# PufferAI/PufferLib

Measured on AMD Instinct MI355X. Metric: env steps/sec end-to-end PPO (rollout+GAE+update), 4096 envs, higher is better.
Workload: dtype f32; 1 GPU; squared d=3 nt=1, 4096 envs/GPU x 128 steps, obs 49->64 f32 rows, MLP 128, 4 minibatches x 4 epochs, bptt 16 (BASELINE configs[1]); global_batch=524288, parallelism=dp1

## Files before the change

### pufferlib_amd/csrc/lane_ops.hpp

```cpp
#pragma once
#include "common.hpp"

namespace pfa {

template <int CTRL>
__device__ __forceinline__ float dpp_f(float x) {
    return __int_as_float(__builtin_amdgcn_update_dpp(0, __float_as_int(x), CTRL, 0xf, 0xf, false));
}
template <int CTRL>
__device__ __forceinline__ int dpp_i(int x) {
    return __builtin_amdgcn_update_dpp(0, x, CTRL, 0xf, 0xf, false);
}

constexpr int kDppXor1 = 0xB1;
constexpr int kDppXor2 = 0x4E;
constexpr int kDppHalfMirror = 0x141;
constexpr int kDppMirror = 0x140;

__device__ __forceinline__ float row16_max(float x) {
    x = fmaxf(x, dpp_f<kDppXor1>(x));
    x = fmaxf(x, dpp_f<kDppXor2>(x));
    x = fmaxf(x, dpp_f<kDppHalfMirror>(x));
    x = fmaxf(x, dpp_f<kDppMirror>(x));
    return x;
}

__device__ __forceinline__ float row16_sum(float x) {
    x = x + dpp_f<kDppXor1>(x);
    x = x + dpp_f<kDppXor2>(x);
    x = x + dpp_f<kDppHalfMirror>(x);
    x = x + dpp_f<kDppMirror>(x);
    return x;
}

__device__ __forceinline__ void row16_argmax(float &best, int &idx) {
#define PFA_ARGMAX_STEP(CTRL)                                   \
    {                                                           \
        const float ob = dpp_f<CTRL>(best);                     \
        const int oi = dpp_i<CTRL>(idx);                        \
        const bool take = (ob > best) | ((ob == best) & (oi < idx));  \
        best = take ? ob : best;                                \
        idx = take ? oi : idx;                                  \
    }
    PFA_ARGMAX_STEP(kDppXor1)
    PFA_ARGMAX_STEP(kDppXor2)
    PFA_ARGMAX_STEP(kDppHalfMirror)
    PFA_ARGMAX_STEP(kDppMirror)
#undef PFA_ARGMAX_STEP
}

}
```

### pufferlib_amd/csrc/rollout.hip

```cpp
#include "common.hpp"
#include "lane_ops.hpp"
#include "mlp_tile.hpp"
#include "philox.hpp"
#include "rollout_tile.hpp"
#include "sampler.hpp"
#include "squared_env.hpp"

namespace pfa {

#ifdef PFA_PROBES
__device__ unsigned long long *g_rtrace = nullptr;
__device__ int g_rtrace_t0 = 0, g_rtrace_steps = 0;
#define PFA_RSTAMP(t, k)                                                                                            \
    do {                                                                                                            \
        if (g_rtrace && blockIdx.x == 0 && (threadIdx.x & 63) == 0 && (t) >= g_rtrace_t0 && (t) < g_rtrace_t0 + g_rtrace_steps) \
            g_rtrace[(((size_t)(threadIdx.x >> 6)) * g_rtrace_steps + ((t) - g_rtrace_t0)) * 8 + (k)] = __builtin_amdgcn_s_memtime(); \
    } while (0)
#else
#define PFA_RSTAMP(t, k) do { } while (0)
#endif

template <int DP, int KS, int MW = kMW>
__global__ void __launch_bounds__(kRollThreads) mlp_forward_sample_kernel(const float *obs, long long rows, MlpView pv,
                                                                         int a, uint32_t heads, const float *noise,
                                                                         uint64_t seed, uint64_t step, long long row_offset,
                                                                         long long *actions, float *logprob, float *entropy,
                                                                         float *value) {
    __shared__ float xs[XTile<DP>::kFloats];
    __shared__ float part[kRollWaves][kPartFloats];
    SliceFrags<DP, KS, MW> w;
    w.load(pv);
    const int le = threadIdx.x >> 4, lo = threadIdx.x & 15;
    const long long tiles = (rows + 15) / 16;
    for (long long tile = blockIdx.x; tile < tiles; tile += gridDim.x) {
        __syncthreads();
        stage_rows<DP>(obs, tile * 16, rows, xs);
        __syncthreads();
        forward_slice<DP, KS, MW>(w, xs, part);
        __syncthreads();
        const long long row = tile * 16 + le;
        const bool ok = row < rows;
        const float q = ok ? noise_lane(noise ? noise + row * a : nullptr, seed, step, (uint64_t)(row_offset + row), lo, a) : 1.0f;
        const LaneSample sm = heads ? sample_lanes_heads(part, le, lo, a, heads, q) : sample_lanes(part, le, lo, a, q);
        if (ok && lo == 0) {
            actions[row] = sm.action;
            logprob[row] = sm.logprob;
            if (entropy) entropy[row] = sm.entropy;
            value[row] = sm.value;
        }
    }
}

template <int DP, int EPW, bool NT1, int KS, int MW = kMW>
__global__ void __launch_bounds__(kRollThreads) rollout_mlp_squared_kernel(SquaredView v, MlpView pv, int a,
                                                                          pfa_experience ex, const float *noise,
                                                                          uint64_t seed, uint64_t step0, long long env_offset,
                                                                          float *live_obs, float *live_rew, uint8_t *live_term,
                                                                          uint8_t *live_trunc, uint8_t *live_mask) {
    constexpr int XS = XTile<DP>::XS;
    __shared__ float xs[XTile<DP>::kFloats];
    __shared__ float part[kRollWaves][kPartFloats];
    __shared__ uint16_t tg[NT1 ? 1 : 16 * kMaxTargets];
    __builtin_amdgcn_s_setprio(3);
    __shared__ RewardTable rtab;
    const int le = threadIdx.x >> 4, lo = threadIdx.x & 15;
    const int e = blockIdx.x * EPW + le;
    const bool env_ok = le < EPW && e < v.n;
    const bool owner = lo == 0 && env_ok;
    const int T = ex.horizon_T;

    SliceFrags<DP, KS, MW> w;
    w.load(pv);

    stage_rows<DP>(live_obs, (long long)blockIdx.x * EPW, v.n, xs, EPW);
    if (NT1) rtab.build(v.d);
    SquaredEnv s;
    Target1 t1;
    float reward = 0.0f;
    bool terminal = false;
    long long filled = 0;
    uint16_t next_cell = 0;
    uint32_t slot = 0;
    const size_t tape_n = (size_t)v.n;
    if (owner) {
        squared_load(v, e, s);
        if (NT1) {
            t1.set(v.tgt[e], v.g);
            filled = v.hdr->rounds_filled;
            slot = s.rounds % (uint32_t)v.tape_rounds;
            next_cell = v.tape[(size_t)slot * tape_n + e];
        } else {
            for (int t = 0; t < v.nt; ++t) tg[le * kMaxTargets + t] = v.tgt[(size_t)t * v.n + e];
        }
        reward = live_rew[e];
        terminal = live_term[e] != 0;
    }
    const bool noise_lane_ok = env_ok && lo < a;
    const float *nz = noise && noise_lane_ok ? noise + (size_t)e * a + lo : nullptr;
    const size_t nz_step = (size_t)v.n * a;
    float q_next = nz ? nz[0] : 1.0f;
    __builtin_amdgcn_s_waitcnt(0x0F70);
    __syncthreads();

    for (int t = 0; t < T; ++t) {
        PFA_RSTAMP(t, 0);
        unstage_rows<DP>(xs, ex.obs + (size_t)t * DP, (long long)blockIdx.x * EPW, v.n, (size_t)T * DP, EPW);
        PFA_RSTAMP(t, 1);
        forward_slice<DP, KS, MW>(w, xs, part);
        PFA_RSTAMP(t, 2);
        lds_barrier();
        PFA_RSTAMP(t, 3);
        const float q = noise ? q_next
                              : (env_ok ? noise_lane(nullptr, seed, step0 + t, (uint64_t)(env_offset + e), lo, a) : 1.0f);
#ifdef PFA_PROBES
        if (q == -12345.678f) PFA_RSTAMP(t, 7);
#endif
        PFA_RSTAMP(t, 4);
        const LaneSample sm = sample_lanes(part, le, lo, a, q);
#ifdef PFA_PROBES
        if (sm.value == 12345.678f) PFA_RSTAMP(t, 7);
#endif
        PFA_RSTAMP(t, 5);
        if (owner) {
            const float stored_reward = reward;
            const bool stored_terminal = terminal;
            float *grid = xs + le * XS;
            if (NT1) {
                if (s.done) {
                    if ((long long)s.rounds >= filled) v.hdr->underrun = 1;
                    squared_reset_nt1(v, s, grid, t1, next_cell, reward, terminal);
                    s.rounds += 1;
                    slot = slot + 1 == (uint32_t)v.tape_rounds ? 0u : slot + 1;
                } else {
                    squared_step_nt1(v, s, grid, t1, rtab, sm.action, reward, terminal);
                }
            } else {
                uint16_t *tc = tg + le * kMaxTargets;
                if (s.done) {
                    if ((long long)s.rounds >= v.hdr->rounds_filled) v.hdr->underrun = 1;
                    const uint16_t *tr = v.tape + (size_t)(s.rounds % (uint32_t)v.tape_rounds) * v.nt * v.n;
                    squared_reset(v, e, s, grid, tr, tc, reward, terminal);
                    s.rounds += 1;
                } else {
                    bool fin;
                    double fr, fs;
                    int fl;
                    squared_step(v, s, grid, tc, sm.action, reward, terminal, fin, fr, fl, fs);
                }
            }
            const size_t row = (size_t)e * T + t;
            ex.rewards[row] = stored_reward;
            ex.dones[row] = stored_terminal ? 1.0f : 0.0f;
            ex.actions[row] = sm.action;
            ex.logprobs[row] = sm.logprob;
            ex.values[row] = sm.value;
            if (NT1) next_cell = v.tape[(size_t)slot * tape_n + e];
        }
        if (nz && t + 1 < T) q_next = nz[(size_t)(t + 1) * nz_step];
        PFA_RSTAMP(t, 6);
        lds_barrier();
        PFA_RSTAMP(t, 7);
    }

    if (owner) {
        squared_store(v, e, s);
        if (NT1) {
            v.tgt[e] = t1.cell;
        } else {
            for (int t = 0; t < v.nt; ++t) v.tgt[(size_t)t * v.n + e] = tg[le * kMaxTargets + t];
        }
        v.fin[e] = 0;
        live_rew[e] = reward;
        live_term[e] = terminal ? 1 : 0;
        live_trunc[e] = 0;
        live_mask[e] = 1;
    }
    unstage_rows<DP>(xs, live_obs, (long long)blockIdx.x * EPW, v.n, (size_t)DP, EPW);
}

__global__ void __launch_bounds__(256) philox_exp_noise_kernel(float *out, long long steps, long long rows, int a, int groups,
                                                               uint64_t seed, uint64_t step0, long long row_offset) {
    const long long total = steps * rows * groups;
    for (long long i = (long long)blockIdx.x * blockDim.x + threadIdx.x; i < total; i += (long long)gridDim.x * blockDim.x) {
        const int j4 = (int)(i % groups);
        const long long tr = i / groups;
        const long long r = tr % rows, t = tr / rows;
        const uint64_t step = step0 + (uint64_t)t, row = (uint64_t)(row_offset + r);
        const u32x4 w = philox4x32_10((uint32_t)row, (uint32_t)j4, (uint32_t)step, (uint32_t)(step >> 32), (uint32_t)seed,
                                      (uint32_t)(seed >> 32));
        float *o = out + (size_t)tr * a + 4 * j4;
        const int left = a - 4 * j4;
        o[0] = -logf(philox_uniform(w.x));
        if (left > 1) o[1] = -logf(philox_uniform(w.y));
        if (left > 2) o[2] = -logf(philox_uniform(w.z));
        if (left > 3) o[3] = -logf(philox_uniform(w.w));
    }
}

struct TilePolicy {
    MlpView pv;
    int obs_dim, obs_stride;
    uint32_t heads;
};

static int check_shape(bool flat, int hidden, int obs_dim, int obs_stride, int a, uint32_t heads) {
    if (flat) {
        PFA_REQUIRE(hidden == kHidden, "mlp: hidden must be %d (got %d)", kHidden, hidden);
    } else {
        PFA_REQUIRE(hidden == 64 || hidden == 128 || hidden == 256 || hidden == 512, "mlp view: hidden %d is not one of 64/128/256/512", hidden);
    }
    PFA_REQUIRE(obs_stride == 16 || obs_stride == 32 || obs_stride == 64 || (flat && (obs_stride == 96 || obs_stride == 128)),
                "mlp: obs_stride must be one of %s (got %d)", flat ? "16/32/64/96/128" : "16/32/64", obs_stride);
    PFA_REQUIRE(obs_dim >= 1 && obs_dim <= obs_stride, "mlp: obs_dim %d out of range", obs_dim);
    PFA_REQUIRE(a >= 1 && a <= 15, "mlp: num_actions must be in 1..15 (got %d)", a);
    PFA_REQUIRE(heads == 0 || (flat && heads_count(heads, a) >= 1), "mlp: head sizes 0x%x do not sum to num_actions %d", heads, a);
    return 0;
}
static int check_dims(const pfa_mlp_dims *d) {
    PFA_REQUIRE(d != nullptr, "mlp: null dims");
    return check_shape(true, d->hidden, d->obs_dim, d->obs_stride, d->num_actions, d->heads);
}
static int check_view(const pfa_mlp_view *p) {
    PFA_REQUIRE(p != nullptr, "mlp view: null");
    PFA_REQUIRE(p->w1 && p->b1 && p->w2 && p->b2 && p->wv && p->bv, "mlp view: null tensor");
    PFA_REQUIRE(p->ldw1 >= p->obs_dim, "mlp view: obs_dim %d / ldw1 %d out of range", p->obs_dim, p->ldw1);
    return check_shape(false, p->hidden, p->obs_dim, p->obs_stride, p->num_actions, 0);
}
static int policy_of_flat(const float *params, const pfa_mlp_dims *d, TilePolicy *out) {
    if (int rc = check_dims(d)) return rc;
    PFA_REQUIRE(params, "mlp: null parameter buffer");
    *out = TilePolicy{mlp_view_of_flat(params, d->obs_stride, d->num_actions), d->obs_dim, d->obs_stride, d->heads};
    return 0;
}
static int policy_of_view(const pfa_mlp_view *p, TilePolicy *out) {
    if (int rc = check_view(p)) return rc;
    *out = TilePolicy{MlpView{p->w1, p->ldw1, p->obs_dim, p->b1, p->w2, p->b2, p->wv, p->bv, p->num_actions, p->hidden}, p->obs_dim,
                      p->obs_stride, 0};
    return 0;
}

template <int DP_, int KS_, int MW_>
struct Tile {
    static constexpr int DP = DP_, KS = KS_, MW = MW_;
};
template <int MW, class Launch>
static void dispatch_stride(const TilePolicy &p, Launch launch) {
    if (p.obs_stride == 64 && p.obs_dim > 48 && p.obs_dim <= 52) return launch(Tile<64, 13, MW>{});
    switch (p.obs_stride) {
        case 16: return launch(Tile<16, 4, MW>{});
        case 32: return launch(Tile<32, 8, MW>{});
        case 64: return launch(Tile<64, 16, MW>{});
    }
    if constexpr (MW == kMW) {
        if (p.obs_stride == 96) return launch(Tile<96, 24, MW>{});
        return launch(Tile<128, 32, MW>{});
    }
}
template <class Launch>
static void dispatch_tile(const TilePolicy &p, Launch launch) {
    switch (p.pv.hidden) {
        case 64: return dispatch_stride<1>(p, launch);
        case 128: return dispatch_stride<2>(p, launch);
        case 256: return dispatch_stride<4>(p, launch);
        default: return dispatch_stride<8>(p, launch);
    }
}

static int launch_forward_sample(const TilePolicy &p, const float *obs, int64_t rows, const float *noise, const pfa_noise_key *key,
                                 int64_t row_offset, int64_t *actions, float *logprob, float *entropy, float *value, pfa_stream_t stream) {
    PFA_REQUIRE(rows >= 0, "mlp.forward: negative rows");
    if (rows == 0) return 0;
    PFA_REQUIRE(obs && actions && logprob && value, "mlp.forward: null buffer");
    PFA_REQUIRE(noise || key, "mlp.forward: need an explicit noise tensor or a Philox key");
    const uint64_t seed = key ? key->seed : 0, step = key ? key->step : 0;
    const int64_t tiles = (rows + 15) / 16;
    const unsigned grid = (unsigned)(tiles < 4096 ? tiles : 4096);
    dispatch_tile(p, [&](auto tile) {
        using T = decltype(tile);
        hipLaunchKernelGGL((mlp_forward_sample_kernel<T::DP, T::KS, T::MW>), dim3(grid), dim3(kRollThreads), 0, (hipStream_t)stream, obs,
                           (long long)rows, p.pv, p.pv.a, p.heads, noise, seed, step, (long long)row_offset, (long long *)actions, logprob,
                           entropy, value);
    });
    PFA_LAUNCH_CHECK();
    return 0;
}

static int launch_rollout_squared(const TilePolicy &p, void *state, const pfa_squared_config *cfg, const pfa_experience *exp,
                                  const float *noise, const pfa_noise_key *key, int64_t env_offset, float *obs, float *rewards,
                                  uint8_t *terminals, uint8_t *truncations, uint8_t *masks, pfa_stream_t stream) {
    PFA_REQUIRE(state && cfg && exp && obs && rewards && terminals && truncations && masks, "rollout: null buffer");
    PFA_REQUIRE(p.heads == 0, "rollout: the fused rollout samples one Discrete head");
    PFA_REQUIRE(cfg->obs_stride == p.obs_stride, "rollout: env obs_stride %d != policy obs_stride %d", cfg->obs_stride, p.obs_stride);
    PFA_REQUIRE(exp->horizon_T >= 1, "rollout: horizon must be >= 1");
    PFA_REQUIRE(exp->obs && exp->actions && exp->logprobs && exp->values && exp->rewards && exp->dones,
                "rollout: null experience buffer");
    PFA_REQUIRE(noise || key, "rollout: need an explicit noise tensor or a Philox key");
    PFA_REQUIRE(cfg->num_targets <= kMaxTargets, "rollout: too many targets");
    SquaredView v = squared_view(state, *cfg);
    const uint64_t seed = key ? key->seed : 0, step = key ? key->step : 0;
    ScopedKernelTimer timer("rollout_mlp_squared", (hipStream_t)stream);
    const unsigned grid = (unsigned)((cfg->num_envs + 15) / 16);
    const bool nt1 = cfg->num_targets == 1;
    dispatch_tile(p, [&](auto tile) {
        using T = decltype(tile);
        auto *kernel = nt1 ? rollout_mlp_squared_kernel<T::DP, 16, true, T::KS, T::MW> : rollout_mlp_squared_kernel<T::DP, 16, false, T::KS, T::MW>;
        hipLaunchKernelGGL(kernel, dim3(grid), dim3(kRollThreads), 0, (hipStream_t)stream, v, p.pv, p.pv.a, *exp, noise, seed, step,
                           (long long)env_offset, obs, rewards, terminals, truncations, masks);
    });
    PFA_LAUNCH_CHECK();
    return 0;
}

}

using namespace pfa;

#ifdef PFA_PROBES
extern "C" int pfa_probe_set_rollout_trace(unsigned long long *buf, int t0, int steps) {
    PFA_CHECK_HIP(hipMemcpyToSymbol(HIP_SYMBOL(g_rtrace), &buf, sizeof(buf)));
    PFA_CHECK_HIP(hipMemcpyToSymbol(HIP_SYMBOL(g_rtrace_t0), &t0, sizeof(t0)));
    PFA_CHECK_HIP(hipMemcpyToSymbol(HIP_SYMBOL(g_rtrace_steps), &steps, sizeof(steps)));
    return 0;
}
#endif

extern "C" int64_t pfa_mlp_param_count(const pfa_mlp_dims *dims) {
    if (check_dims(dims)) return -1;
    return mlp_offsets(dims->obs_stride, dims->num_actions).count;
}

extern "C" int pfa_mlp_forward_sample(const float *obs, int64_t rows, const float *params, const pfa_mlp_dims *dims,
                                      const float *noise, const pfa_noise_key *key, int64_t row_offset, int64_t *actions,
                                      float *logprob, float *entropy, float *value, pfa_stream_t stream) {
    TilePolicy p;
    if (int rc = policy_of_flat(params, dims, &p)) return rc;
    return launch_forward_sample(p, obs, rows, noise, key, row_offset, actions, logprob, entropy, value, stream);
}

extern "C" int pfa_mlp_view_supported(const pfa_mlp_view *p) { return check_view(p) == 0 ? 1 : 0; }

extern "C" int pfa_mlp_view_forward_sample(const float *obs, int64_t rows, const pfa_mlp_view *view, const float *noise,
                                           const pfa_noise_key *key, int64_t row_offset, int64_t *actions, float *logprob,
                                           float *entropy, float *value, pfa_stream_t stream) {
    TilePolicy p;
    if (int rc = policy_of_view(view, &p)) return rc;
    return launch_forward_sample(p, obs, rows, noise, key, row_offset, actions, logprob, entropy, value, stream);
}

extern "C" int pfa_philox_exp_noise(float *out, int64_t steps, int64_t rows, int32_t num_actions, const pfa_noise_key *key,
                                    int64_t row_offset, pfa_stream_t stream) {
    PFA_REQUIRE(steps >= 0 && rows >= 0, "philox noise: negative shape");
    PFA_REQUIRE(num_actions >= 1 && num_actions <= 15, "philox noise: num_actions must be in 1..15 (got %d)", num_actions);
    if (steps == 0 || rows == 0) return 0;
    PFA_REQUIRE(out && key, "philox noise: null buffer");
    const int groups = (num_actions + 3) / 4;
    const long long total = (long long)steps * rows * groups;
    const unsigned grid = (unsigned)((total + 255) / 256 < 65536 ? (total + 255) / 256 : 65536);
    ScopedKernelTimer timer("philox_exp_noise", (hipStream_t)stream);
    hipLaunchKernelGGL(philox_exp_noise_kernel, dim3(grid), dim3(256), 0, (hipStream_t)stream, out, (long long)steps, (long long)rows,
                       (int)num_actions, groups, key->seed, key->step, (long long)row_offset);
    PFA_LAUNCH_CHECK();
    return 0;
}

extern "C" int pfa_rollout_mlp_squared(void *state, const pfa_squared_config *cfg, const float *params,
                                       const pfa_mlp_dims *dims, const pfa_experience *exp, const float *noise,
                                       const pfa_noise_key *key, int64_t env_offset, float *obs, float *rewards,
                                       uint8_t *terminals, uint8_t *truncations, uint8_t *masks, pfa_stream_t stream) {
    TilePolicy p;
    if (int rc = policy_of_flat(params, dims, &p)) return rc;
    return launch_rollout_squared(p, state, cfg, exp, noise, key, env_offset, obs, rewards, terminals, truncations, masks, stream);
}

extern "C" int pfa_rollout_mlp_view_squared(void *state, const pfa_squared_config *cfg, const pfa_mlp_view *view, const pfa_experience *exp,
                                            const float *noise, const pfa_noise_key *key, int64_t env_offset, float *obs, float *rewards,
                                            uint8_t *terminals, uint8_t *truncations, uint8_t *masks, pfa_stream_t stream) {
    TilePolicy p;
    if (int rc = policy_of_view(view, &p)) return rc;
    return launch_rollout_squared(p, state, cfg, exp, noise, key, env_offset, obs, rewards, terminals, truncations, masks, stream);
}
```

### pufferlib_amd/csrc/rollout_tile.hpp

```cpp
#pragma once
#include "common.hpp"
#include "lane_ops.hpp"
#include "mlp_tile.hpp"
#include "philox.hpp"
#include "sampler.hpp"

namespace pfa {

constexpr int kRollThreads = 256;
constexpr int kRollWaves = 4;
constexpr int kMW = kMT / kRollWaves;

struct MlpView {
    const float *w1;
    int ldw1, cols;
    const float *b1;
    const float *w2;
    const float *b2;
    const float *wv;
    const float *bv;
    int a, hidden;
    __device__ __forceinline__ float w2v(int o, int u) const { return o < a ? w2[o * hidden + u] : (o == a ? wv[u] : 0.0f); }
    __device__ __forceinline__ float b2v(int o) const { return o < a ? b2[o] : (o == a ? bv[0] : 0.0f); }
};
inline MlpView mlp_view_of_flat(const float *params, int dp, int a) {
    const MlpOffsets off = mlp_offsets(dp, a);
    return MlpView{params + off.w1, dp, dp, params + off.b1, params + off.w2, params + off.b2, params + off.wv, params + off.bv, a, kHidden};
}

template <int DP, int KS = DP / 4, int MW = kMW>
struct SliceFrags {
    float w1f[MW][KS], b1f[MW][4], w2f[MW][4], bo[4];
    __device__ __forceinline__ void load(const float *params, int a) {
        const MlpOffsets off = mlp_offsets(DP, a);
        const int wv = wave_id(), c = lane_id() & 15, g = lane_id() >> 4;
#pragma unroll
        for (int i = 0; i < MW; ++i) {
            const int m = MW * wv + i;
#pragma unroll
            for (int kk = 0; kk < KS; ++kk) w1f[i][kk] = params[off.w1 + (16 * m + c) * DP + 4 * kk + g];
#pragma unroll
            for (int r = 0; r < 4; ++r) {
                b1f[i][r] = params[off.b1 + 16 * m + 4 * g + r];
                w2f[i][r] = w2v_at(params, off, a, c, 16 * m + 4 * g + r);
            }
        }
#pragma unroll
        for (int r = 0; r < 4; ++r) bo[r] = wv == 0 ? b2v_at(params, off, a, 4 * g + r) : 0.0f;
    }
    __device__ __forceinline__ void load(const MlpView &p) {
        const int wv = wave_id(), c = lane_id() & 15, g = lane_id() >> 4;
#pragma unroll
        for (int i = 0; i < MW; ++i) {
            const int m = MW * wv + i;
#pragma unroll
            for (int kk = 0; kk < KS; ++kk) w1f[i][kk] = 4 * kk + g < p.cols ? p.w1[(size_t)(16 * m + c) * p.ldw1 + 4 * kk + g] : 0.0f;
#pragma unroll
            for (int r = 0; r < 4; ++r) {
                b1f[i][r] = p.b1[16 * m + 4 * g + r];
                w2f[i][r] = p.w2v(c, 16 * m + 4 * g + r);
            }
        }
#pragma unroll
        for (int r = 0; r < 4; ++r) bo[r] = wv == 0 ? p.b2v(4 * g + r) : 0.0f;
    }
};

template <int DP>
__device__ __forceinline__ void stage_rows(const float *src, long long first_row, long long rows, float *xs,
                                           int tile_rows = 16) {
    constexpr int XS = XTile<DP>::XS, V = DP / 4;
    for (int idx = threadIdx.x; idx < 16 * V; idx += kRollThreads) {
        const int r = idx / V, c4 = idx - r * V;
        float4 x = make_float4(0.f, 0.f, 0.f, 0.f);
        if (r < tile_rows && first_row + r < rows) x = *reinterpret_cast<const float4 *>(src + (first_row + r) * DP + 4 * c4);
        float2 *d = reinterpret_cast<float2 *>(xs + r * XS + 4 * c4);
        d[0] = make_float2(x.x, x.y);
        d[1] = make_float2(x.z, x.w);
    }
}

template <int DP>
__device__ __forceinline__ void unstage_rows(const float *xs, float *dst, long long first_row, long long rows, size_t row_stride,
                                             int tile_rows = 16) {
    constexpr int XS = XTile<DP>::XS, V = DP / 4;
    for (int idx = threadIdx.x; idx < tile_rows * V; idx += kRollThreads) {
        const int r = idx / V, c4 = idx - r * V;
        if (first_row + r < rows) {
            const float2 *sp = reinterpret_cast<const float2 *>(xs + r * XS + 4 * c4);
            const float2 lo2 = sp[0], hi2 = sp[1];
            *reinterpret_cast<float4 *>(dst + (size_t)(first_row + r) * row_stride + 4 * c4) = make_float4(lo2.x, lo2.y, hi2.x, hi2.y);
        }
    }
}

template <int DP, int KS = DP / 4, int MW = kMW>
__device__ __forceinline__ void forward_slice(const SliceFrags<DP, KS, MW> &w, const float *xs, float (*part)[kPartFloats]) {
    constexpr int XS = XTile<DP>::XS;
    const int wv = wave_id(), c = lane_id() & 15, g = lane_id() >> 4;
    f32x4 h[MW];
#pragma unroll
    for (int i = 0; i < MW; ++i) h[i] = f32x4{w.b1f[i][0], w.b1f[i][1], w.b1f[i][2], w.b1f[i][3]};
    float bv[KS];
#pragma unroll
    for (int kk = 0; kk < KS; ++kk) bv[kk] = xs[c * XS + 4 * kk + g];
    __builtin_amdgcn_sched_barrier(0);
#pragma unroll
    for (int kk = 0; kk < KS; ++kk) {
#pragma unroll
        for (int i = 0; i < MW; ++i) h[i] = mfma16(w.w1f[i][kk], bv[kk], h[i]);
    }
    f32x4 o0 = f32x4{w.bo[0], w.bo[1], w.bo[2], w.bo[3]}, o1 = f32x4{0.f, 0.f, 0.f, 0.f};
#pragma unroll
    for (int i = 0; i < MW; i += 2) {
#pragma unroll
        for (int r = 0; r < 4; ++r) {
            o0 = mfma16(w.w2f[i][r], fmaxf(h[i][r], 0.0f), o0);
            if constexpr (MW >= 2) o1 = mfma16(w.w2f[i + 1][r], fmaxf(h[i + 1][r], 0.0f), o1);
        }
    }
    const f32x4 po = o0 + o1;
#pragma unroll
    for (int r = 0; r < 4; ++r) part[wv][(4 * g + r) * kPartStride + c] = po[r];
}

__device__ __forceinline__ LaneSample sample_lanes(const float (*part)[kPartFloats], int le, int lo, int a, float q) {
    const int i = lo * kPartStride + le;
    const float mine = (part[0][i] + part[1][i]) + (part[2][i] + part[3][i]);
    return sample_row16(mine, lo, a, q);
}
__device__ __forceinline__ LaneSample sample_lanes_heads(const float (*part)[kPartFloats], int le, int lo, int a, uint32_t heads, float q) {
    const int i = lo * kPartStride + le;
    const float mine = (part[0][i] + part[1][i]) + (part[2][i] + part[3][i]);
    return sample_row16_heads(mine, lo, a, heads, q);
}

}
```

Measured before the change: 422.1 million env_steps/s.

## Overlap obs unstaging with first-layer MFMAs and tighten DPP/relu lane ops

The per-step obs write-out (LDS to global) is split into a load phase issued alongside the activation reads and a store phase placed inside the first-layer MFMA loop between sched barriers. The goal is to hide global-store issue behind matrix work rather than run it serially before the forward pass. It also replaces update_dpp with mov_dpp using bound_ctrl, rewrites row16_max as inline fused v_max_f32_dpp asm with s_nops, and computes ReLU as an integer max on the float bits. The inline asm and the integer ReLU change handling of NaN and negative zero, and the extra staged registers can raise register pressure.

After: 426.3 million env_steps/s, median of 6. Within noise of the previous version (+1.0%).

```diff
diff --git a/pufferlib_amd/csrc/lane_ops.hpp b/pufferlib_amd/csrc/lane_ops.hpp
--- a/pufferlib_amd/csrc/lane_ops.hpp
+++ b/pufferlib_amd/csrc/lane_ops.hpp
@@ -5,11 +5,11 @@
 
 template <int CTRL>
 __device__ __forceinline__ float dpp_f(float x) {
-    return __int_as_float(__builtin_amdgcn_update_dpp(0, __float_as_int(x), CTRL, 0xf, 0xf, false));
+    return __int_as_float(__builtin_amdgcn_mov_dpp(__float_as_int(x), CTRL, 0xf, 0xf, true));
 }
 template <int CTRL>
 __device__ __forceinline__ int dpp_i(int x) {
-    return __builtin_amdgcn_update_dpp(0, x, CTRL, 0xf, 0xf, false);
+    return __builtin_amdgcn_mov_dpp(x, CTRL, 0xf, 0xf, true);
 }
 
 constexpr int kDppXor1 = 0xB1;
@@ -18,10 +18,16 @@
 constexpr int kDppMirror = 0x140;
 
 __device__ __forceinline__ float row16_max(float x) {
-    x = fmaxf(x, dpp_f<kDppXor1>(x));
-    x = fmaxf(x, dpp_f<kDppXor2>(x));
-    x = fmaxf(x, dpp_f<kDppHalfMirror>(x));
-    x = fmaxf(x, dpp_f<kDppMirror>(x));
+    asm("s_nop 1\n\t"
+        "v_max_f32_dpp %0, %0, %0 quad_perm:[1,0,3,2] row_mask:0xf bank_mask:0xf bound_ctrl:1\n\t"
+        "s_nop 1\n\t"
+        "v_max_f32_dpp %0, %0, %0 quad_perm:[2,3,0,1] row_mask:0xf bank_mask:0xf bound_ctrl:1\n\t"
+        "s_nop 1\n\t"
+        "v_max_f32_dpp %0, %0, %0 row_half_mirror row_mask:0xf bank_mask:0xf bound_ctrl:1\n\t"
+        "s_nop 1\n\t"
+        "v_max_f32_dpp %0, %0, %0 row_mirror row_mask:0xf bank_mask:0xf bound_ctrl:1\n\t"
+        "s_nop 1"
+        : "+v"(x));
     return x;
 }
 
diff --git a/pufferlib_amd/csrc/rollout.hip b/pufferlib_amd/csrc/rollout.hip
--- a/pufferlib_amd/csrc/rollout.hip
+++ b/pufferlib_amd/csrc/rollout.hip
@@ -104,9 +104,9 @@
 
     for (int t = 0; t < T; ++t) {
         PFA_RSTAMP(t, 0);
-        unstage_rows<DP>(xs, ex.obs + (size_t)t * DP, (long long)blockIdx.x * EPW, v.n, (size_t)T * DP, EPW);
+        RowUnstage<DP> rows_out(xs, ex.obs + (size_t)t * DP, (long long)blockIdx.x * EPW, v.n, (size_t)T * DP, EPW);
         PFA_RSTAMP(t, 1);
-        forward_slice<DP, KS, MW>(w, xs, part);
+        forward_slice<DP, KS, MW>(w, xs, part, rows_out);
         PFA_RSTAMP(t, 2);
         lds_barrier();
         PFA_RSTAMP(t, 3);
diff --git a/pufferlib_amd/csrc/rollout_tile.hpp b/pufferlib_amd/csrc/rollout_tile.hpp
--- a/pufferlib_amd/csrc/rollout_tile.hpp
+++ b/pufferlib_amd/csrc/rollout_tile.hpp
@@ -1,4 +1,5 @@
 #pragma once
+#include <type_traits>
 #include "common.hpp"
 #include "lane_ops.hpp"
 #include "mlp_tile.hpp"
@@ -81,22 +82,53 @@
 }
 
 template <int DP>
+struct RowUnstage {
+    static constexpr int XS = XTile<DP>::XS, V = DP / 4, kPieces = (16 * V + kRollThreads - 1) / kRollThreads;
+    float *dst;
+    long long first_row, rows;
+    size_t row_stride;
+    int tile_rows;
+    const float *xs;
+    float2 lo2[kPieces], hi2[kPieces];
+    __device__ __forceinline__ RowUnstage(const float *xs_, float *dst_, long long first_row_, long long rows_, size_t row_stride_,
+                                          int tile_rows_ = 16)
+        : dst(dst_), first_row(first_row_), rows(rows_), row_stride(row_stride_), tile_rows(tile_rows_), xs(xs_) {}
+    __device__ __forceinline__ bool live(int idx, int r) const { return idx < tile_rows * V && first_row + r < rows; }
+    __device__ __forceinline__ void load() {
+#pragma unroll
+        for (int i = 0; i < kPieces; ++i) {
+            const int idx = threadIdx.x + i * kRollThreads, r = idx / V, c4 = idx - r * V;
+            if (live(idx, r)) {
+                const float2 *sp = reinterpret_cast<const float2 *>(xs + r * XS + 4 * c4);
+                lo2[i] = sp[0];
+                hi2[i] = sp[1];
+            }
+        }
+    }
+    __device__ __forceinline__ void store() const {
+#pragma unroll
+        for (int i = 0; i < kPieces; ++i) {
+            const int idx = threadIdx.x + i * kRollThreads, r = idx / V, c4 = idx - r * V;
+            if (live(idx, r))
+                *reinterpret_cast<float4 *>(dst + (size_t)(first_row + r) * row_stride + 4 * c4) = make_float4(lo2[i].x, lo2[i].y, hi2[i].x, hi2[i].y);
+        }
+    }
+};
+template <int DP>
 __device__ __forceinline__ void unstage_rows(const float *xs, float *dst, long long first_row, long long rows, size_t row_stride,
                                              int tile_rows = 16) {
-    constexpr int XS = XTile<DP>::XS, V = DP / 4;
-    for (int idx = threadIdx.x; idx < tile_rows * V; idx += kRollThreads) {
-        const int r = idx / V, c4 = idx - r * V;
-        if (first_row + r < rows) {
-            const float2 *sp = reinterpret_cast<const float2 *>(xs + r * XS + 4 * c4);
-            const float2 lo2 = sp[0], hi2 = sp[1];
-            *reinterpret_cast<float4 *>(dst + (size_t)(first_row + r) * row_stride + 4 * c4) = make_float4(lo2.x, lo2.y, hi2.x, hi2.y);
-        }
-    }
+    RowUnstage<DP> u(xs, dst, first_row, rows, row_stride, tile_rows);
+    u.load();
+    u.store();
 }
+struct NoUnstage {};
 
-template <int DP, int KS = DP / 4, int MW = kMW>
-__device__ __forceinline__ void forward_slice(const SliceFrags<DP, KS, MW> &w, const float *xs, float (*part)[kPartFloats]) {
+__device__ __forceinline__ float relu_bits(float x) { return __int_as_float(max(__float_as_int(x), 0)); }
+
+template <int DP, int KS = DP / 4, int MW = kMW, class Side = NoUnstage>
+__device__ __forceinline__ void forward_slice(const SliceFrags<DP, KS, MW> &w, const float *xs, float (*part)[kPartFloats], Side &&side = Side{}) {
     constexpr int XS = XTile<DP>::XS;
+    constexpr bool kSide = !std::is_same<std::decay_t<Side>, NoUnstage>::value;
     const int wv = wave_id(), c = lane_id() & 15, g = lane_id() >> 4;
     f32x4 h[MW];
 #pragma unroll
@@ -104,19 +136,27 @@
     float bv[KS];
 #pragma unroll
     for (int kk = 0; kk < KS; ++kk) bv[kk] = xs[c * XS + 4 * kk + g];
+    if constexpr (kSide) side.load();
     __builtin_amdgcn_sched_barrier(0);
 #pragma unroll
     for (int kk = 0; kk < KS; ++kk) {
 #pragma unroll
         for (int i = 0; i < MW; ++i) h[i] = mfma16(w.w1f[i][kk], bv[kk], h[i]);
+        if constexpr (kSide) {
+            if (kk == 1) {
+                __builtin_amdgcn_sched_barrier(0);
+                side.store();
+                __builtin_amdgcn_sched_barrier(0);
+            }
+        }
     }
     f32x4 o0 = f32x4{w.bo[0], w.bo[1], w.bo[2], w.bo[3]}, o1 = f32x4{0.f, 0.f, 0.f, 0.f};
 #pragma unroll
     for (int i = 0; i < MW; i += 2) {
 #pragma unroll
         for (int r = 0; r < 4; ++r) {
-            o0 = mfma16(w.w2f[i][r], fmaxf(h[i][r], 0.0f), o0);
-            if constexpr (MW >= 2) o1 = mfma16(w.w2f[i + 1][r], fmaxf(h[i + 1][r], 0.0f), o1);
+            o0 = mfma16(w.w2f[i][r], relu_bits(h[i][r]), o0);
+            if constexpr (MW >= 2) o1 = mfma16(w.w2f[i + 1][r], relu_bits(h[i + 1][r]), o1);
         }
     }
     const f32x4 po = o0 + o1;
```
